# bigai-nlco/VideoTGB

Measured on AMD Instinct MI355X. Metric: clips/sec end-to-end VideoQA (96->8 frames), higher is better.
Workload: dtype bf16; 1 GPU; InstructBLIP-Vicuna-7B + TGB, T=96->8 of 32 frames, 224x224, greedy 16 new tokens (BASELINE.json configs[2]); inputs=resident in HBM when the timed region starts, global_batch=124, parallelism=clip-parallel x1 (no data-path collective), streams=1, weights=seeded N(0,0.02) random init

## Files before the change

### videotgb_amd/csrc/conv64.hip

```cpp
#include <type_traits>
#include <utility>
#include "common.h"
#include "pair_h8.h"

namespace {

constexpr int C64_R = 8, C64_RS = 128;
constexpr int C64_ROW_BYTES = C64_RS * 128;
constexpr int C64_LDS = C64_R * C64_ROW_BYTES + 8 * 32 * 2 * 4 + 64 * 4;
typedef __attribute__((address_space(3))) void* c64_lptr_t;

struct Conv64Params {
    const bf16_t* in;
    const bf16_t* w;
    const float* bias;
    float* out_f32;
    float* stats;
    float* stats_part;
    bf16_t* out_bf16;
    const bf16_t* resid;
    int n_img, H, W, relu, post_relu;
    int parts, rows_per_part;
};

template <int MODE>
__global__ __launch_bounds__(512) void conv3x3_c64_kernel(const Conv64Params p) {
#if defined(__HIP_DEVICE_COMPILE__)
    extern __shared__ __attribute__((aligned(16))) char ring[];
    float* const xch = reinterpret_cast<float*>(ring + C64_R * C64_ROW_BYTES);
    const int tid = threadIdx.x, lane = tid & 63, fr = lane & 15, fg = lane >> 4;
    const int wave = __builtin_amdgcn_readfirstlane(tid >> 6);
    const int wm = wave & 3, wn = wave >> 2;
    const int H = p.H, W = p.W;

    bf16x8 wf[9][2][2];
#pragma unroll
    for (int t = 0; t < 9; t++)
#pragma unroll
        for (int ks = 0; ks < 2; ks++)
#pragma unroll
            for (int i = 0; i < 2; i++)
                wf[t][ks][i] = *reinterpret_cast<const bf16x8*>(p.w + (wn * 32 + i * 16 + fr) * 576 + t * 64 + ks * 32 + fg * 8);
    float* const bias_s = xch + 8 * 32 * 2;
    if (tid < 64) bias_s[tid] = p.bias[tid];

    unsigned dma_off[2];
#pragma unroll
    for (int q = 0; q < 2; q++) {
        const int slot = (wave * 2 + q) * 8 + (lane >> 3), x = slot - 1, c = (lane & 7) ^ ((slot >> 1) & 7);
        dma_off[q] = (x >= 0 && x < W) ? (unsigned)(x * 64 + c * 8) * 2u : 0x80000000u;
    }
    unsigned x_off[3];
    int px[2];
#pragma unroll
    for (int j = 0; j < 2; j++) px[j] = wm * 32 + j * 16 + fr;
#pragma unroll
    for (int kx = 0; kx < 3; kx++) x_off[kx] = (unsigned)((px[0] + kx) * 128 + ((fg ^ (((px[0] + kx) >> 1) & 7)) << 4));

    typedef __attribute__((__vector_size__(4 * sizeof(unsigned)))) unsigned u32x4_t;
    typedef __attribute__((__vector_size__(2 * sizeof(unsigned)))) unsigned u32x2_t;
    constexpr unsigned OOB = 0x80000000u;
    constexpr int ES = MODE == 0 ? 4 : 2;
    unsigned o_off[2][2];
#pragma unroll
    for (int i = 0; i < 2; i++)
#pragma unroll
        for (int j = 0; j < 2; j++) o_off[i][j] = px[j] < W ? (unsigned)(px[j] * 64 + wn * 32 + i * 16 + fg * 4) * ES : OOB;

    const int n_units = p.n_img * p.parts;
    for (int unit = blockIdx.x; unit < n_units; unit += gridDim.x) {
        const int img = unit / p.parts, y0 = (unit - img * p.parts) * p.rows_per_part;
        if (y0 >= H) continue;
        const int y1 = y0 + p.rows_per_part < H ? y0 + p.rows_per_part : H;
        const bf16_t* const ibase = p.in + (int64_t)img * H * W * 64;
        const auto rsrc = __builtin_amdgcn_make_buffer_rsrc(const_cast<bf16_t*>(ibase), 0, H * W * 128, 0x00020000);
        const auto orsrc = __builtin_amdgcn_make_buffer_rsrc(MODE == 0 ? (void*)(p.out_f32 + (int64_t)img * H * W * 64) : (void*)(p.out_bf16 + (int64_t)img * H * W * 64), 0,
                                                             H * W * 64 * ES, 0x00020000);
        const auto rrsrc = __builtin_amdgcn_make_buffer_rsrc(const_cast<bf16_t*>(p.resid ? p.resid + (int64_t)img * H * W * 64 : ibase), 0, H * W * 128, 0x00020000);
#define C64_ISSUE(yy)                                                                                                          \
        {                                                                                                                      \
            const int so_ = ((yy) >= 0 && (yy) < H) ? (yy) * W * 128 : 0x7FFFFF00;        \
            char* const dst_ = ring + ((yy) & (C64_R - 1)) * C64_ROW_BYTES + (wave * 2) * 1024;                                \
            __builtin_amdgcn_raw_ptr_buffer_load_lds(rsrc, (c64_lptr_t)dst_, 16, dma_off[0], so_, 0, 0);                       \
            __builtin_amdgcn_raw_ptr_buffer_load_lds(rsrc, (c64_lptr_t)(dst_ + 1024), 16, dma_off[1], so_, 0, 0);              \
        }
        __builtin_amdgcn_s_waitcnt(0x0F70);
        __builtin_amdgcn_s_barrier();
        C64_ISSUE(y0 - 1)
        C64_ISSUE(y0)
        C64_ISSUE(y0 + 1)
        C64_ISSUE(y0 + 2)
        f32x4 s1[2] = {f32x4{0.f, 0.f, 0.f, 0.f}, f32x4{0.f, 0.f, 0.f, 0.f}}, s2[2] = {s1[0], s1[0]};
        for (int y = y0; y < y1; y += 2) {
            if (y == y0) __builtin_amdgcn_s_waitcnt(0x0F70);
            else __builtin_amdgcn_s_waitcnt(0x0F78);
            __builtin_amdgcn_s_barrier();
            bf16x4 rres[2][2][2];
            if constexpr (MODE == 1) {
                if (p.resid) {
#pragma unroll
                    for (int o = 0; o < 2; o++)
#pragma unroll
                        for (int i = 0; i < 2; i++)
#pragma unroll
                            for (int j = 0; j < 2; j++) {
                                const unsigned off = (y + o < y1 && o_off[i][j] != OOB) ? o_off[i][j] + (unsigned)((y + o) * W * 64 * 2) : OOB;
                                rres[o][i][j] = __builtin_bit_cast(bf16x4, __builtin_amdgcn_raw_buffer_load_b64(rrsrc, off, 0, 0));
                            }
                }
            }
            C64_ISSUE(y + 3)
            C64_ISSUE(y + 4)
            f32x4 acc[2][2][2];
#pragma unroll
            for (int o = 0; o < 2; o++)
#pragma unroll
                for (int i = 0; i < 2; i++)
#pragma unroll
                    for (int j = 0; j < 2; j++) acc[o][i][j] = f32x4{0.f, 0.f, 0.f, 0.f};
#pragma unroll
            for (int rr = 0; rr < 4; rr++) {
                const char* const rowp = ring + ((y + rr - 1) & (C64_R - 1)) * C64_ROW_BYTES;
#pragma unroll
                for (int kx = 0; kx < 3; kx++)
#pragma unroll
                    for (int ks = 0; ks < 2; ks++) {
                        const bf16x8 x0 = *reinterpret_cast<const bf16x8*>(rowp + (x_off[kx] ^ (ks * 64)));
                        const bf16x8 x1 = *reinterpret_cast<const bf16x8*>(rowp + (x_off[kx] ^ (ks * 64)) + 2048);
#pragma unroll
                        for (int o = 0; o < 2; o++) {
                            const int ky = rr - o;
                            if (ky < 0 || ky > 2) continue;
#pragma unroll
                            for (int i = 0; i < 2; i++) {
                                acc[o][i][0] = __builtin_amdgcn_mfma_f32_16x16x32_bf16(wf[ky * 3 + kx][ks][i], x0, acc[o][i][0], 0, 0, 0);
                                acc[o][i][1] = __builtin_amdgcn_mfma_f32_16x16x32_bf16(wf[ky * 3 + kx][ks][i], x1, acc[o][i][1], 0, 0, 0);
                            }
                        }
                    }
            }
            f32x4 b4[2];
#pragma unroll
            for (int i = 0; i < 2; i++) b4[i] = *reinterpret_cast<const f32x4*>(bias_s + wn * 32 + i * 16 + fg * 4);
#pragma unroll
            for (int o = 0; o < 2; o++) {
                const bool row_ok = y + o < y1;
#pragma unroll
                for (int i = 0; i < 2; i++)
#pragma unroll
                    for (int j = 0; j < 2; j++) {
                        const bool ok = row_ok && o_off[i][j] != OOB;
                        const unsigned off = ok ? o_off[i][j] + (unsigned)((y + o) * W * 64 * ES) : OOB;
                        f32x4 v = acc[o][i][j] + b4[i];
                        if constexpr (MODE == 0) {
                            __builtin_amdgcn_raw_buffer_store_b128(__builtin_bit_cast(u32x4_t, v), orsrc, off, 0, 0);
                            const f32x4 vz = {ok ? v[0] : 0.f, ok ? v[1] : 0.f, ok ? v[2] : 0.f, ok ? v[3] : 0.f};
                            s1[i] += vz;
                            s2[i] += vz * vz;
                        } else {
                            if (p.relu) v = f32x4{fmaxf(v[0], 0.f), fmaxf(v[1], 0.f), fmaxf(v[2], 0.f), fmaxf(v[3], 0.f)};
                            if (p.resid) {
                                const bf16x4 r = rres[o][i][j];
                                v += f32x4{(float)r[0], (float)r[1], (float)r[2], (float)r[3]};
                            }
                            if (p.post_relu) v = f32x4{fmaxf(v[0], 0.f), fmaxf(v[1], 0.f), fmaxf(v[2], 0.f), fmaxf(v[3], 0.f)};
                            const bf16x4 pk = {(bf16_t)v[0], (bf16_t)v[1], (bf16_t)v[2], (bf16_t)v[3]};
                            __builtin_amdgcn_raw_buffer_store_b64(__builtin_bit_cast(u32x2_t, pk), orsrc, off, 0, 0);
                        }
                    }
            }
        }
#undef C64_ISSUE
        if constexpr (MODE == 0) {
#pragma unroll
            for (int i = 0; i < 2; i++)
#pragma unroll
                for (int e = 0; e < 4; e++) {
                    float a_ = s1[i][e], b_ = s2[i][e];
#pragma unroll
                    for (int off = 1; off < 16; off <<= 1) { a_ += __shfl_xor(a_, off); b_ += __shfl_xor(b_, off); }
                    s1[i][e] = a_; s2[i][e] = b_;
                }
            __builtin_amdgcn_s_waitcnt(0xC07F);
            __builtin_amdgcn_s_barrier();
            if (fr == 0) {
#pragma unroll
                for (int i = 0; i < 2; i++)
#pragma unroll
                    for (int e = 0; e < 4; e++) {
                        xch[(wave * 32 + i * 16 + fg * 4 + e) * 2] = s1[i][e];
                        xch[(wave * 32 + i * 16 + fg * 4 + e) * 2 + 1] = s2[i][e];
                    }
            }
            __syncthreads();
            if (tid < 128) {
                const int ch = tid >> 1, which = tid & 1, wn_ = ch >> 5, c32 = ch & 31;
                float t = 0.f;
#pragma unroll
                for (int m_ = 0; m_ < 4; m_++) t += xch[((wn_ * 4 + m_) * 32 + c32) * 2 + which];
                if (p.parts == 1) p.stats[((int64_t)img * 64 + ch) * 2 + which] = t;
                else p.stats_part[((int64_t)unit * 64 + ch) * 2 + which] = t;
            }
        }
    }
#endif
}


constexpr int ST_R = 5;
struct StemParams {
    const float* img;
    const bf16_t* w;
    const float* bias;
    float* out_f32;
    float* stats;
    float* stats_part;
    bf16_t* out_bf16;
    int n_img, H, W, relu;
    int parts, rows_per_part;
    int h8;
};

template <int MODE, bool X3>
__global__ __launch_bounds__(512) void stem7x7_kernel(const StemParams p) {
    static_assert(X3 ? (MODE == 0 || MODE == 2) : (MODE == 0 || MODE == 1), "stem7x7: bf16 stores fp32 / bf16 rows, the split form fp32 / pair rows");
#if defined(__HIP_DEVICE_COMPILE__)
    extern __shared__ __attribute__((aligned(16))) char ring[];
    const int tid = threadIdx.x, lane = tid & 63, fr = lane & 15, fg = lane >> 4;
    const int wave = __builtin_amdgcn_readfirstlane(tid >> 6);
    const int wm = wave & 3, wn = wave >> 2;
    const int H = p.H, W = p.W, H2 = H >> 1, W2 = W >> 1;
    const int row_bytes = W2 * 256;
    float* const xch = reinterpret_cast<float*>(ring + ST_R * row_bytes);
    float* const bias_s = xch + 8 * 32 * 2;
    if (tid < 64) bias_s[tid] = p.bias[tid];
    for (int i = tid; i < ST_R * W2 * 4; i += 512) {
        const int pxl = i >> 2, X = pxl % W2, c = 6 + (i & 1) + ((i & 2) << 2);
        *reinterpret_cast<uint4*>(ring + pxl * 256 + ((c ^ (X & 15)) << 4)) = make_uint4(0, 0, 0, 0);
    }
    constexpr int W_LD = X3 ? 768 : 512;
    bf16x8 wf[16][2];
#pragma unroll
    for (int s_ = 0; s_ < 16; s_++)
#pragma unroll
        for (int i = 0; i < 2; i++)
            wf[s_][i] = *reinterpret_cast<const bf16x8*>(p.w + (wn * 32 + i * 16 + fr) * W_LD + (X3 ? (s_ >> 3) * 512 + (s_ & 7) * 32 : s_ * 32) + fg * 8);
    const bool builder = tid < W2 * 4;
    const int bX = tid >> 2, bdX = tid & 3, bcol = 2 * (bX + bdX - 2);
    const bool bcol_ok = builder && bcol >= 0 && bcol + 1 < W;
    const int bcol_c = bcol < 0 ? 0 : bcol + 1 < W ? bcol : W - 2;
    unsigned b_off[3];
#pragma unroll
    for (int q = 0; q < 3; q++) {
        const int off = bdX * 24 + q * 8;
        b_off[q] = (unsigned)(bX * 256 + (((off >> 4) ^ (bX & 15)) << 4) + (off & 8));
    }
    int px[2];
    unsigned x_off[2];
#pragma unroll
    for (int j = 0; j < 2; j++) {
        px[j] = wm * 32 + j * 16 + fr;
        const int pc = px[j] < W2 ? px[j] : 0;
        x_off[j] = (unsigned)(pc * 256 + ((fg ^ (pc & 15)) << 4));
    }
    typedef __attribute__((__vector_size__(4 * sizeof(unsigned)))) unsigned u32x4_t;
    typedef __attribute__((__vector_size__(2 * sizeof(unsigned)))) unsigned u32x2_t;
    constexpr unsigned OOB = 0x80000000u;
    constexpr int ES = MODE == 0 ? 4 : 2;
    constexpr int PXU = MODE == 2 ? 128 : 64;
    unsigned o_off[2][2];
#pragma unroll
    for (int i = 0; i < 2; i++)
#pragma unroll
        for (int j = 0; j < 2; j++) o_off[i][j] = px[j] < W2 ? (unsigned)(px[j] * PXU + wn * 32 + i * 16 + fg * 4) * ES : OOB;

    const int n_units = p.n_img * p.parts;
    for (int unit = blockIdx.x; unit < n_units; unit += gridDim.x) {
        const int img = unit / p.parts, y0 = (unit - img * p.parts) * p.rows_per_part;
        if (y0 >= H2) continue;
        const int y1 = y0 + p.rows_per_part < H2 ? y0 + p.rows_per_part : H2;
        const float* const ibase = p.img + (int64_t)img * 3 * H * W;
        const auto orsrc = __builtin_amdgcn_make_buffer_rsrc(MODE == 0 ? (void*)(p.out_f32 + (int64_t)img * H2 * W2 * 64) : (void*)(p.out_bf16 + (int64_t)img * H2 * W2 * PXU),
                                                             0, H2 * W2 * PXU * ES, 0x00020000);
        float2 ld[6];
#define ST_LOAD(Yp)       \
        {                                                                                                    \
            const int yc_ = (Yp) < 0 ? 0 : (Yp) >= H2 ? H2 - 1 : (Yp);                                       \
            _Pragma("unroll") for (int py = 0; py < 2; py++)                                                 \
                _Pragma("unroll") for (int c = 0; c < 3; c++)                                                \
                    ld[py * 3 + c] = *reinterpret_cast<const float2*>(ibase + ((int64_t)c * H + 2 * yc_ + py) * W + bcol_c); \
        }
#define ST_WRITE(Yp)                                                                                         \
        if (builder) {                                                                                       \
            const bool in_ = bcol_ok && (Yp) >= 0 && (Yp) < H2;                                              \
            bf16_t hi[12], lo[12];                                                                           \
            _Pragma("unroll") for (int py = 0; py < 2; py++)                                                 \
                _Pragma("unroll") for (int c = 0; c < 3; c++) {                                              \
                    const float d0 = in_ ? ld[py * 3 + c].x - 127.5f : 0.f, d1 = in_ ? ld[py * 3 + c].y - 127.5f : 0.f; \
                    const float h0_ = bf16_round(d0), h1_ = bf16_round(d1);                                  \
                    hi[py * 6 + c] = (bf16_t)h0_; lo[py * 6 + c] = (bf16_t)(d0 - h0_);                       \
                    hi[py * 6 + 3 + c] = (bf16_t)h1_; lo[py * 6 + 3 + c] = (bf16_t)(d1 - h1_);               \
                }                                                                                            \
            char* const rb_ = ring + ((((Yp) % ST_R) + ST_R) % ST_R) * row_bytes;                            \
            _Pragma("unroll") for (int q = 0; q < 3; q++) {                                                  \
                *reinterpret_cast<bf16x4*>(rb_ + b_off[q]) = bf16x4{hi[q * 4], hi[q * 4 + 1], hi[q * 4 + 2], hi[q * 4 + 3]}; \
                *reinterpret_cast<bf16x4*>(rb_ + (b_off[q] ^ 128)) = bf16x4{lo[q * 4], lo[q * 4 + 1], lo[q * 4 + 2], lo[q * 4 + 3]}; \
            }                                                                                                \
        }
        __syncthreads();
        for (int yy = y0 - 2; yy <= y0 + 1; yy++) {
            ST_LOAD(yy)
            ST_WRITE(yy)
        }
        f32x4 s1[2] = {f32x4{0.f, 0.f, 0.f, 0.f}, f32x4{0.f, 0.f, 0.f, 0.f}}, s2[2] = {s1[0], s1[0]};
        for (int y = y0; y < y1; y++) {
            __builtin_amdgcn_sched_barrier(0);
            __builtin_amdgcn_s_waitcnt(0xC07F);
            __builtin_amdgcn_s_barrier();
            __builtin_amdgcn_sched_barrier(0);
            ST_LOAD(y + 2)
            f32x4 acc[2][2], b4[2];
#define ST_STEP(tY, hl, half, s_)                                                                            \
            {                                                                                                \
                const char* const rowp = ring + ((y + (tY) - 2 + ST_R) % ST_R) * row_bytes;                  \
                const unsigned cx = (unsigned)(((hl) * 8 + (half) * 4) << 4);       \
                const bf16x8 x0 = *reinterpret_cast<const bf16x8*>(rowp + (x_off[0] ^ cx));                  \
                const bf16x8 x1 = *reinterpret_cast<const bf16x8*>(rowp + (x_off[1] ^ cx));                  \
                _Pragma("unroll") for (int i = 0; i < 2; i++) {                                              \
                    acc[i][0] = __builtin_amdgcn_mfma_f32_16x16x32_bf16(wf[s_][i], x0, acc[i][0], 0, 0, 0);  \
                    acc[i][1] = __builtin_amdgcn_mfma_f32_16x16x32_bf16(wf[s_][i], x1, acc[i][1], 0, 0, 0);  \
                }                                                                                            \
            }
            if constexpr (X3) {
#pragma unroll
                for (int i = 0; i < 2; i++) b4[i] = *reinterpret_cast<const f32x4*>(bias_s + wn * 32 + i * 16 + fg * 4);
#pragma unroll
                for (int i = 0; i < 2; i++)
#pragma unroll
                    for (int j = 0; j < 2; j++) acc[i][j] = b4[i] + f32x4{0.f, 0.f, 0.f, 0.f};
#pragma unroll
                for (int c = 0; c < 3; c++) {
#pragma unroll
                    for (int tY = 0; tY < 4; tY++)
#pragma unroll
                        for (int half = 0; half < 2; half++) ST_STEP(tY, c == 1 ? 1 : 0, half, (c == 2 ? 8 : 0) + tY * 2 + half)
                    if (c < 2) __builtin_amdgcn_sched_barrier(0);
                }
            } else {
#pragma unroll
                for (int i = 0; i < 2; i++)
#pragma unroll
                    for (int j = 0; j < 2; j++) acc[i][j] = f32x4{0.f, 0.f, 0.f, 0.f};
#pragma unroll
                for (int tY = 0; tY < 4; tY++)
#pragma unroll
                    for (int hl = 0; hl < 2; hl++)
#pragma unroll
                        for (int half = 0; half < 2; half++) ST_STEP(tY, hl, half, hl * 8 + tY * 2 + half)
#pragma unroll
                for (int i = 0; i < 2; i++) b4[i] = *reinterpret_cast<const f32x4*>(bias_s + wn * 32 + i * 16 + fg * 4);
            }
#undef ST_STEP
#pragma unroll
            for (int i = 0; i < 2; i++)
#pragma unroll
                for (int j = 0; j < 2; j++) {
                    const bool ok = o_off[i][j] != OOB;
                    const unsigned off = ok ? o_off[i][j] + (unsigned)(y * W2 * PXU * ES) : OOB;
                    f32x4 v = X3 ? acc[i][j] : acc[i][j] + b4[i];
                    if constexpr (MODE == 0) {
                        __builtin_amdgcn_raw_buffer_store_b128(__builtin_bit_cast(u32x4_t, v), orsrc, off, 0, 0);
                        const f32x4 vz = {ok ? v[0] : 0.f, ok ? v[1] : 0.f, ok ? v[2] : 0.f, ok ? v[3] : 0.f};
                        s1[i] += vz;
                        s2[i] += vz * vz;
                    } else if constexpr (MODE == 2) {
                        if (p.relu) v = f32x4{fmaxf(v[0], 0.f), fmaxf(v[1], 0.f), fmaxf(v[2], 0.f), fmaxf(v[3], 0.f)};
                        u32x2_t hu, lu;
                        if (p.h8) {
                            h8_split4(v, hu, lu);
                        } else {
                            bf16x4 hi, lo;
                            pair_split4(v, hi, lo);
                            hu = __builtin_bit_cast(u32x2_t, hi); lu = __builtin_bit_cast(u32x2_t, lo);
                        }
                        __builtin_amdgcn_raw_buffer_store_b64(hu, orsrc, off, 0, 0);
                        __builtin_amdgcn_raw_buffer_store_b64(lu, orsrc, ok ? off + 128u : OOB, 0, 0);
                    } else {
                        if (p.relu) v = f32x4{fmaxf(v[0], 0.f), fmaxf(v[1], 0.f), fmaxf(v[2], 0.f), fmaxf(v[3], 0.f)};
                        const bf16x4 pk = {(bf16_t)v[0], (bf16_t)v[1], (bf16_t)v[2], (bf16_t)v[3]};
                        __builtin_amdgcn_raw_buffer_store_b64(__builtin_bit_cast(u32x2_t, pk), orsrc, off, 0, 0);
                    }
                }
            ST_WRITE(y + 2)
        }
#undef ST_LOAD
#undef ST_WRITE
        if constexpr (X3) {
            if (!p.stats) continue;
        }
        if constexpr (MODE == 0) {
#pragma unroll
            for (int i = 0; i < 2; i++)
#pragma unroll
                for (int e = 0; e < 4; e++) {
                    float a_ = s1[i][e], b_ = s2[i][e];
#pragma unroll
                    for (int off = 1; off < 16; off <<= 1) { a_ += __shfl_xor(a_, off); b_ += __shfl_xor(b_, off); }
                    s1[i][e] = a_; s2[i][e] = b_;
                }
            __syncthreads();
            if (fr == 0) {
#pragma unroll
                for (int i = 0; i < 2; i++)
#pragma unroll
                    for (int e = 0; e < 4; e++) {
                        xch[(wave * 32 + i * 16 + fg * 4 + e) * 2] = s1[i][e];
                        xch[(wave * 32 + i * 16 + fg * 4 + e) * 2 + 1] = s2[i][e];
                    }
            }
            __syncthreads();
            if (tid < 128) {
                const int ch = tid >> 1, which = tid & 1, wn_ = ch >> 5, c32 = ch & 31;
                float t = 0.f;
#pragma unroll
                for (int m_ = 0; m_ < 4; m_++) t += xch[((wn_ * 4 + m_) * 32 + c32) * 2 + which];
                if (p.parts == 1) p.stats[((int64_t)img * 64 + ch) * 2 + which] = t;
                else p.stats_part[((int64_t)unit * 64 + ch) * 2 + which] = t;
            }
        }
    }
#endif
}

constexpr int L1_R = 4;
constexpr int L1_MAX_W = 112;
constexpr int L1_READ_SPAN = 130 * 256;
typedef int l1_i32x4 __attribute__((ext_vector_type(4)));
typedef int l1_i32x8 __attribute__((ext_vector_type(8)));
typedef _Float16 l1_f16x8 __attribute__((ext_vector_type(8)));

template <class F, int... G>
__device__ __forceinline__ void l1_static_for(std::integer_sequence<int, G...>, F&& f) { (f(std::integral_constant<int, G>{}), ...); }

struct Layer1H8Params {
    const char* in;
    const char* w;
    const float* bias;
    const int* scale;
    float* out_f32;
    char* out_pair;
    const char* resid;
    int n_img, H, W, out_bf16;
    int parts, rows_per_part, row_bytes;
};

template <int MODE, int OBF>
__global__ __launch_bounds__(512) void layer1_h8_kernel(const Layer1H8Params p) {
#if defined(__HIP_DEVICE_COMPILE__)
    extern __shared__ __attribute__((aligned(16))) char ring[];
    const int tid = threadIdx.x, lane = tid & 63, fr = lane & 15, fg = lane >> 4;
    const int wave = __builtin_amdgcn_readfirstlane(tid >> 6);
    const int wn = wave & 3, wm = wave >> 2;
    const int H = p.H, W = p.W, row_bytes = p.row_bytes;
    const int sc_w = *p.scale;

    l1_i32x4 wh[9][2];
    l1_i32x8 wc[9];
    {
        const char* const wrow = p.w + (wn * 16 + fr) * 2304 + fg * 16;
#pragma unroll
        for (int t = 0; t < 9; t++) {
            wh[t][0] = *reinterpret_cast<const l1_i32x4*>(wrow + t * 128);
            wh[t][1] = *reinterpret_cast<const l1_i32x4*>(wrow + t * 128 + 64);
            wc[t].lo = *reinterpret_cast<const l1_i32x4*>(wrow + (9 + t) * 128);
            wc[t].hi = *reinterpret_cast<const l1_i32x4*>(wrow + (9 + t) * 128 + 64);
        }
    }
    float* const bias_s = reinterpret_cast<float*>(ring + (L1_R - 1) * row_bytes + L1_READ_SPAN);
    if (tid < 64) bias_s[tid] = p.bias[tid];
    __syncthreads();

    constexpr unsigned OOB = 0x80000000u;
    const int n_pieces = row_bytes >> 10;
    const int dma_x = wave * 4 + (lane >> 4) - 1;
    const unsigned dma_off0 = (unsigned)(dma_x * 256 + (((lane & 15) ^ ((dma_x + 1) & 15)) << 4));
    unsigned x_off[3];
#pragma unroll
    for (int kx = 0; kx < 3; kx++) {
        const int slot = wm * 64 + fr + kx;
        x_off[kx] = (unsigned)(slot * 256 + ((fg ^ (slot & 15)) << 4));
    }
    const int nj = W - wm * 64 >= 64 ? 4 : W - wm * 64 <= 0 ? 0 : (W - wm * 64 + 15) >> 4;
    typedef __attribute__((__vector_size__(4 * sizeof(unsigned)))) unsigned u32x4_t;
    typedef __attribute__((__vector_size__(2 * sizeof(unsigned)))) unsigned u32x2_t;
    constexpr int OPX = 256;
    constexpr int OCH = MODE == 0 ? 4 : 2;
    const int px0 = wm * 64 + fr;
    const unsigned o_off0 = (unsigned)(px0 * OPX + (wn * 16 + fg * 4) * OCH);

    const int n_units = p.n_img * p.parts;
    for (int unit = blockIdx.x; unit < n_units; unit += gridDim.x) {
        const int img = unit / p.parts, y0 = (unit - img * p.parts) * p.rows_per_part;
        if (y0 >= H) continue;
        const int y1 = y0 + p.rows_per_part < H ? y0 + p.rows_per_part : H;
        const int64_t ioff = (int64_t)img * H * W * 256;
        const auto rsrc = __builtin_amdgcn_make_buffer_rsrc(const_cast<char*>(p.in + ioff), 0, H * W * 256, 0x00020000);
        const auto orsrc = __builtin_amdgcn_make_buffer_rsrc(MODE == 0 ? (void*)(reinterpret_cast<char*>(p.out_f32) + ioff) : (void*)(p.out_pair + ioff), 0, H * W * OPX, 0x00020000);
        const auto rrsrc = __builtin_amdgcn_make_buffer_rsrc(const_cast<char*>((MODE == 2 ? p.resid : p.in) + ioff), 0, H * W * 256, 0x00020000);
#define L1_ISSUE(yy)                                                                                                          \
        {                                                                                                                      \
            const int so_ = ((yy) >= 0 && (yy) < H) ? (yy) * W * 256 : 0x7FFFFF00;        \
            char* const dst_ = ring + ((yy) & (L1_R - 1)) * row_bytes + wave * 1024;                                           \
            _Pragma("unroll") for (int q = 0; q < 4; q++)                                                                      \
                if (q * 8 + wave < n_pieces)                                                                                   \
                    __builtin_amdgcn_raw_ptr_buffer_load_lds(rsrc, (c64_lptr_t)(dst_ + q * 8192), 16,                          \
                                                             (dma_x + q * 32 >= 0 && dma_x + q * 32 < W) ? dma_off0 + q * 8192u : OOB, so_, 0, 0); \
        }
        __builtin_amdgcn_s_waitcnt(0x0F70);
        __builtin_amdgcn_s_barrier();
        L1_ISSUE(y0 - 1)
        L1_ISSUE(y0)
        L1_ISSUE(y0 + 1)
        auto step = [&](auto nj_c, const int y) {
            constexpr int NJ = decltype(nj_c)::value;
            constexpr int NST = (MODE == 0 ? 1 : 2) * NJ;
            if (y == y0) __builtin_amdgcn_s_waitcnt(0x0F70);
            else __builtin_amdgcn_s_waitcnt(0x0F70 | NST);
            __builtin_amdgcn_s_barrier();
            u32x2_t rh[NJ], rl[NJ];
            if constexpr (MODE == 2) {
#pragma unroll
                for (int jj = 0; jj < NJ; jj++) {
                    const unsigned off = px0 + jj * 16 < W ? o_off0 + (unsigned)(jj * 16 * OPX + y * W * 256) : OOB;
                    rh[jj] = __builtin_bit_cast(u32x2_t, __builtin_amdgcn_raw_buffer_load_b64(rrsrc, off, 0, 0));
                    rl[jj] = __builtin_bit_cast(u32x2_t, __builtin_amdgcn_raw_buffer_load_b64(rrsrc, off != OOB ? off + 128u : OOB, 0, 0));
                }
            }
            L1_ISSUE(y + 2)
            f32x4 acc[NJ];
#pragma unroll
            for (int jj = 0; jj < NJ; jj++) acc[jj] = *reinterpret_cast<const f32x4*>(bias_s + wn * 16 + fg * 4);
            l1_i32x4 xg[3][NJ];
#define L1_READ(g)                                                                                                             \
            {                                                                                                                  \
                constexpr int t_ = (g) < 18 ? (g) / 2 : ((g) - 18) / 2;                                                        \
                constexpr unsigned cx_ = (g) < 18 ? ((g) & 1) * 64u : 128u + ((g) & 1) * 64u;                                  \
                const char* const rowp_ = ring + ((y + t_ / 3 - 1) & (L1_R - 1)) * row_bytes;                                  \
                _Pragma("unroll") for (int jj = 0; jj < NJ; jj++)                                                              \
                    xg[(g) % 3][jj] = *reinterpret_cast<const l1_i32x4*>(rowp_ + (x_off[t_ % 3] ^ cx_) + jj * 4096);           \
            }
            L1_READ(0)
            __builtin_amdgcn_sched_barrier(0);
            l1_static_for(std::make_integer_sequence<int, 36>{}, [&](auto gc) {
                constexpr int g = decltype(gc)::value;
                if constexpr (g + 1 < 36) { L1_READ(g + 1) }
                if constexpr (g < 18) {
#pragma unroll
                    for (int jj = 0; jj < NJ; jj++)
                        acc[jj] = __builtin_amdgcn_mfma_f32_16x16x32_f16(__builtin_bit_cast(l1_f16x8, wh[g / 2][g & 1]), __builtin_bit_cast(l1_f16x8, xg[g % 3][jj]), acc[jj], 0, 0, 0);
                } else if constexpr ((g & 1) != 0) {
#pragma unroll
                    for (int jj = 0; jj < NJ; jj++) {
                        l1_i32x8 xc;
                        xc.lo = xg[(g - 1) % 3][jj]; xc.hi = xg[g % 3][jj];
                        acc[jj] = __builtin_amdgcn_mfma_scale_f32_16x16x128_f8f6f4(wc[(g - 18) / 2], xc, acc[jj], 0, 1, 0, sc_w, 0, 127);
                    }
                }
                if constexpr (g + 1 < 36) __builtin_amdgcn_sched_group_barrier(0x100, NJ, 0);
                if constexpr (g < 18 || (g & 1) != 0) __builtin_amdgcn_sched_group_barrier(0x008, NJ, 0);
                __builtin_amdgcn_sched_barrier(0);
            });
#undef L1_READ
            __builtin_amdgcn_sched_barrier(0);
#pragma unroll
            for (int jj = 0; jj < NJ; jj++) {
                const bool ok = px0 + jj * 16 < W;
                const unsigned off = ok ? o_off0 + (unsigned)(jj * 16 * OPX + y * W * OPX) : OOB;
                f32x4 v = acc[jj];
                if constexpr (MODE == 0) {
                    __builtin_amdgcn_raw_buffer_store_b128(__builtin_bit_cast(u32x4_t, v), orsrc, off, 0, 0);
                } else {
                    v = f32x4{fmaxf(v[0], 0.f), fmaxf(v[1], 0.f), fmaxf(v[2], 0.f), fmaxf(v[3], 0.f)};
                    if constexpr (MODE == 2) {
                        v += h8_join4(rh[jj], rl[jj]);
                        v = f32x4{fmaxf(v[0], 0.f), fmaxf(v[1], 0.f), fmaxf(v[2], 0.f), fmaxf(v[3], 0.f)};
                    }
                    u32x2_t hu, lu;
                    if constexpr (OBF) {
                        bf16x4 hi, lo;
                        pair_split4(v, hi, lo);
                        hu = __builtin_bit_cast(u32x2_t, hi); lu = __builtin_bit_cast(u32x2_t, lo);
                    } else {
                        h8_split4(v, hu, lu);
                    }
                    __builtin_amdgcn_raw_buffer_store_b64(hu, orsrc, off, 0, 0);
                    __builtin_amdgcn_raw_buffer_store_b64(lu, orsrc, ok ? off + 128u : OOB, 0, 0);
                }
            }
        };
        if (nj == 3) {
            for (int y = y0; y < y1; y++) step(std::integral_constant<int, 3>{}, y);
        } else {
            for (int y = y0; y < y1; y++) step(std::integral_constant<int, 4>{}, y);
        }
#undef L1_ISSUE
    }
#endif
}

}

bool conv3x3_c64_supported(int H, int W) { return W >= 16 && W <= C64_RS - 2 && H >= 1; }

size_t conv64_stats_part_floats(int n_img) { return ((size_t)n_img + 4 * (size_t)cu_count()) * 2 * 64 * 2; }

int launch_conv3x3_c64(const void* in, const void* w, const float* bias, float* out_f32, float* stats, float* stats_part, void* out_bf16, const void* resid,
                       int n_img, int H, int W, int relu, int post_relu, hipStream_t s) {
    VTGB_REQUIRE(conv3x3_c64_supported(H, W), VTGB_EUNSUPPORTED, "conv3x3_c64: W=%d outside [16, %d]", W, C64_RS - 2);
    VTGB_REQUIRE((int64_t)H * W * 128 < 0x7FFFFF00ll, VTGB_EUNSUPPORTED, "conv3x3_c64: image too large");
    Conv64Params p;
    p.in = (const bf16_t*)in; p.w = (const bf16_t*)w; p.bias = bias; p.out_f32 = out_f32; p.stats = stats; p.stats_part = stats_part; p.out_bf16 = (bf16_t*)out_bf16;
    p.resid = (const bf16_t*)resid; p.n_img = n_img; p.H = H; p.W = W; p.relu = relu; p.post_relu = post_relu;
    int parts = 1;
    while ((int64_t)n_img * parts < 4 * cu_count() && H / (parts * 2) >= 8) parts *= 2;
    p.rows_per_part = 2 * ((H + 2 * parts - 1) / (2 * parts));
    p.parts = (H + p.rows_per_part - 1) / p.rows_per_part;
    const int64_t units = (int64_t)n_img * p.parts;
    const int grid = units < cu_count() ? (int)units : cu_count();
    if (out_f32 && p.parts > 1) VTGB_REQUIRE(stats_part && (size_t)units * 128 <= conv64_stats_part_floats(n_img), VTGB_EINVAL, "conv3x3_c64: partial-moment scratch missing");
    const double flops = 2.0 * n_img * H * W * 64.0 * 576.0;
    ProfScope prof(VTGB_PROF_CONV, flops, s, flops);
    static DeviceOnce a0, a1;
    if (out_f32) {
        VTGB_REQUIRE(stats, VTGB_EINVAL, "conv3x3_c64: fp32 output needs the moments buffer");
        VTGB_FUNC_LDS_ONCE(a0, conv3x3_c64_kernel<0>, C64_LDS);
        hipLaunchKernelGGL(conv3x3_c64_kernel<0>, dim3(grid), dim3(512), C64_LDS, s, p);
        if (p.parts > 1) VTGB_TRY(launch_stats_finish_parts(stats_part, stats, n_img, p.parts, 64, s));
    } else {
        VTGB_FUNC_LDS_ONCE(a1, conv3x3_c64_kernel<1>, C64_LDS);
        hipLaunchKernelGGL(conv3x3_c64_kernel<1>, dim3(grid), dim3(512), C64_LDS, s, p);
    }
    VTGB_HIP(hipGetLastError());
    return VTGB_OK;
}

bool stem7x7_supported(int H, int W) { return (H % 2) == 0 && (W % 2) == 0 && W / 2 >= 16 && W / 2 <= 112 && H / 2 >= 4; }

static int stem7x7_launch(bool x3, const float* img, const void* w, const float* bias, float* out_f32, float* stats, float* stats_part, void* out16, int h8, int n_img,
                          int H, int W, int relu, hipStream_t s) {
    VTGB_REQUIRE(stem7x7_supported(H, W), VTGB_EUNSUPPORTED, "stem7x7: %d x %d unsupported", H, W);
    const int H2 = H / 2, W2 = W / 2;
    VTGB_REQUIRE((int64_t)H2 * W2 * 256 < 0x7FFFFF00ll, VTGB_EUNSUPPORTED, "stem7x7: image too large");
    StemParams p;
    p.img = img; p.w = (const bf16_t*)w; p.bias = bias; p.out_f32 = out_f32; p.stats = stats; p.stats_part = stats_part; p.out_bf16 = (bf16_t*)out16;
    p.n_img = n_img; p.H = H; p.W = W; p.relu = relu; p.h8 = h8;
    int parts = 1;
    while ((int64_t)n_img * parts < 4 * cu_count() && H2 / (parts * 2) >= 14) parts *= 2;
    p.rows_per_part = (H2 + parts - 1) / parts;
    p.parts = (H2 + p.rows_per_part - 1) / p.rows_per_part;
    const int64_t units = (int64_t)n_img * p.parts;
    const int grid = units < cu_count() ? (int)units : cu_count();
    if (out_f32 && stats && p.parts > 1)
        VTGB_REQUIRE(stats_part && (size_t)units * 128 <= conv64_stats_part_floats(n_img), VTGB_EINVAL, "stem7x7: partial-moment scratch missing");
    const int lds = ST_R * W2 * 256 + 8 * 32 * 2 * 4 + 64 * 4;
    constexpr int lds_max = ST_R * 112 * 256 + 8 * 32 * 2 * 4 + 64 * 4;
    const double flops = 2.0 * n_img * H2 * W2 * 64.0 * 147.0, exec = 2.0 * n_img * H2 * W2 * 64.0 * (x3 ? 768.0 : 512.0);
    ProfScope prof(VTGB_PROF_CONV, flops, s, exec);
    static DeviceOnce a0, a1, a2, a3;
    if (out_f32) {
        VTGB_REQUIRE(stats || x3, VTGB_EINVAL, "stem7x7: fp32 output needs the moments buffer");
        if (x3) {
            VTGB_FUNC_LDS_ONCE(a2, (stem7x7_kernel<0, true>), lds_max);
            hipLaunchKernelGGL((stem7x7_kernel<0, true>), dim3(grid), dim3(512), lds, s, p);
        } else {
            VTGB_FUNC_LDS_ONCE(a0, (stem7x7_kernel<0, false>), lds_max);
            hipLaunchKernelGGL((stem7x7_kernel<0, false>), dim3(grid), dim3(512), lds, s, p);
        }
        if (stats && p.parts > 1) VTGB_TRY(launch_stats_finish_parts(stats_part, stats, n_img, p.parts, 64, s));
    } else if (x3) {
        VTGB_FUNC_LDS_ONCE(a3, (stem7x7_kernel<2, true>), lds_max);
        hipLaunchKernelGGL((stem7x7_kernel<2, true>), dim3(grid), dim3(512), lds, s, p);
    } else {
        VTGB_FUNC_LDS_ONCE(a1, (stem7x7_kernel<1, false>), lds_max);
        hipLaunchKernelGGL((stem7x7_kernel<1, false>), dim3(grid), dim3(512), lds, s, p);
    }
    VTGB_HIP(hipGetLastError());
    return VTGB_OK;
}

int launch_stem7x7(const float* img, const void* w, const float* bias, float* out_f32, float* stats, float* stats_part, void* out_bf16, int n_img, int H, int W,
                   int relu, hipStream_t s) {
    return stem7x7_launch(false, img, w, bias, out_f32, stats, stats_part, out_bf16, 0, n_img, H, W, relu, s);
}
int launch_stem7x7_x3(const float* img, const void* w, const float* bias, float* out_f32, float* stats, float* stats_part, void* out_pair, int h8, int n_img, int H,
                      int W, hipStream_t s) {
    VTGB_REQUIRE((out_f32 != nullptr) != (out_pair != nullptr), VTGB_EINVAL, "stem7x7 x3: exactly one of the fp32 rows and the pair rows");
    return stem7x7_launch(true, img, w, bias, out_f32, stats, stats_part, out_pair, h8, n_img, H, W, out_pair ? 1 : 0, s);
}

bool layer1_h8_supported(int H, int W) { return W >= 16 && W <= L1_MAX_W && H >= 4 && (int64_t)H * W * 256 < 0x7FFFFF00ll; }

int launch_layer1_h8(const void* in, const void* w, const float* bias, const int* scale, float* out_f32, void* out_pair, const void* resid, int out_bf16, int n_img, int H,
                     int W, hipStream_t s) {
    VTGB_REQUIRE(n_img > 0 && layer1_h8_supported(H, W), VTGB_EUNSUPPORTED, "layer1_h8: %d images of %d x %d outside 16 <= W <= %d, H >= 4", n_img, H, W, L1_MAX_W);
    VTGB_REQUIRE(in && w && bias && scale && ((out_f32 != nullptr) != (out_pair != nullptr)) && (!resid || out_pair) && (!out_bf16 || resid), VTGB_EINVAL,
                 "layer1_h8: operands, the scale byte and exactly one of the fp32 rows and the pair rows (resid belongs to pair rows, bf16 pairs to the residual tail)");
    Layer1H8Params p;
    p.in = (const char*)in; p.w = (const char*)w; p.bias = bias; p.scale = scale; p.out_f32 = out_f32; p.out_pair = (char*)out_pair; p.resid = (const char*)resid;
    p.n_img = n_img; p.H = H; p.W = W; p.out_bf16 = out_bf16;
    p.row_bytes = ((W + 2 + 3) / 4) * 1024;
    int parts = 1;
    while ((int64_t)n_img * parts < 4 * cu_count() && H / (parts * 2) >= 7) parts *= 2;
    p.rows_per_part = (H + parts - 1) / parts;
    p.parts = (H + p.rows_per_part - 1) / p.rows_per_part;
    const int64_t units = (int64_t)n_img * p.parts;
    const int grid = units < cu_count() ? (int)units : cu_count();
    const int lds = (L1_R - 1) * p.row_bytes + L1_READ_SPAN + 256;
    constexpr int lds_max = (L1_R - 1) * ((L1_MAX_W + 2 + 3) / 4) * 1024 + L1_READ_SPAN + 256;
    const double flops = 2.0 * n_img * H * W * 64.0 * 576.0;
    ProfScope prof(VTGB_PROF_CONV, flops, s, 2.0 * flops);
    static DeviceOnce a0, a1, a2, a3;
    if (out_f32) {
        VTGB_FUNC_LDS_ONCE(a0, (layer1_h8_kernel<0, 0>), lds_max);
        hipLaunchKernelGGL((layer1_h8_kernel<0, 0>), dim3(grid), dim3(512), lds, s, p);
    } else if (!resid) {
        VTGB_FUNC_LDS_ONCE(a1, (layer1_h8_kernel<1, 0>), lds_max);
        hipLaunchKernelGGL((layer1_h8_kernel<1, 0>), dim3(grid), dim3(512), lds, s, p);
    } else if (!out_bf16) {
        VTGB_FUNC_LDS_ONCE(a2, (layer1_h8_kernel<2, 0>), lds_max);
        hipLaunchKernelGGL((layer1_h8_kernel<2, 0>), dim3(grid), dim3(512), lds, s, p);
    } else {
        VTGB_FUNC_LDS_ONCE(a3, (layer1_h8_kernel<2, 1>), lds_max);
        hipLaunchKernelGGL((layer1_h8_kernel<2, 1>), dim3(grid), dim3(512), lds, s, p);
    }
    VTGB_HIP(hipGetLastError());
    return VTGB_OK;
}
```

Before: 38.67 clips/s.

## Add 4-wave layer1 h8 conv kernel for the non-residual modes

```diff
diff --git a/videotgb_amd/csrc/conv64.hip b/videotgb_amd/csrc/conv64.hip
--- a/videotgb_amd/csrc/conv64.hip
+++ b/videotgb_amd/csrc/conv64.hip
@@ -597,6 +597,149 @@
                     __builtin_amdgcn_raw_buffer_store_b64(lu, orsrc, ok ? off + 128u : OOB, 0, 0);
                 }
             }
+        };
+        if (nj == 3) {
+            for (int y = y0; y < y1; y++) step(std::integral_constant<int, 3>{}, y);
+        } else {
+            for (int y = y0; y < y1; y++) step(std::integral_constant<int, 4>{}, y);
+        }
+#undef L1_ISSUE
+    }
+#endif
+}
+
+constexpr int l1_waitcnt_vm(int n) { return 0x0F70 | (n & 15) | ((n >> 4) << 14); }
+
+template <int MODE>
+__global__ __launch_bounds__(256) __attribute__((amdgpu_waves_per_eu(1, 1))) void layer1_h8_w4_kernel(const Layer1H8Params p) {
+    static_assert(MODE == 0 || MODE == 1, "layer1_h8_w4: fp32 rows or relu(.) as an f16c8 pair (the residual tail runs on layer1_h8_kernel)");
+#if defined(__HIP_DEVICE_COMPILE__)
+    extern __shared__ __attribute__((aligned(16))) char ring[];
+    const int tid = threadIdx.x, lane = tid & 63, fr = lane & 15, fg = lane >> 4;
+    const int wave = __builtin_amdgcn_readfirstlane(tid >> 6);
+    const int cp = wave & 1, wm = wave >> 1;
+    const int H = p.H, W = p.W, row_bytes = p.row_bytes;
+    const int sc_w = *p.scale;
+
+    l1_i32x4 wh[2][9][2];
+    l1_i32x8 wc[2][9];
+    f32x4 bias[2];
+#pragma unroll
+    for (int b = 0; b < 2; b++) {
+        const char* const wrow = p.w + (cp * 32 + b * 16 + fr) * 2304 + fg * 16;
+#pragma unroll
+        for (int t = 0; t < 9; t++) {
+            wh[b][t][0] = *reinterpret_cast<const l1_i32x4*>(wrow + t * 128);
+            wh[b][t][1] = *reinterpret_cast<const l1_i32x4*>(wrow + t * 128 + 64);
+            wc[b][t].lo = *reinterpret_cast<const l1_i32x4*>(wrow + (9 + t) * 128);
+            wc[b][t].hi = *reinterpret_cast<const l1_i32x4*>(wrow + (9 + t) * 128 + 64);
+        }
+        bias[b] = *reinterpret_cast<const f32x4*>(p.bias + cp * 32 + b * 16 + fg * 4);
+    }
+
+    constexpr unsigned OOB = 0x80000000u;
+    const int n_pieces = row_bytes >> 10;
+    const int dma_x = wave * 4 + (lane >> 4) - 1;
+    const unsigned dma_off0 = (unsigned)(dma_x * 256 + (((lane & 15) ^ ((dma_x + 1) & 15)) << 4));
+    unsigned x_off[3];
+#pragma unroll
+    for (int kx = 0; kx < 3; kx++) {
+        const int slot = wm * 64 + fr + kx;
+        x_off[kx] = (unsigned)(slot * 256 + ((fg ^ (slot & 15)) << 4));
+    }
+    const int nj = W - wm * 64 >= 64 ? 4 : W - wm * 64 <= 0 ? 0 : (W - wm * 64 + 15) >> 4;
+    typedef __attribute__((__vector_size__(4 * sizeof(unsigned)))) unsigned u32x4_t;
+    typedef __attribute__((__vector_size__(2 * sizeof(unsigned)))) unsigned u32x2_t;
+    constexpr int OPX = 256;
+    constexpr int OCH = MODE == 0 ? 4 : 2;
+    const int px0 = wm * 64 + fr;
+    const unsigned o_off0 = (unsigned)(px0 * OPX + (cp * 32 + fg * 4) * OCH);
+
+    const int n_units = p.n_img * p.parts;
+    for (int unit = blockIdx.x; unit < n_units; unit += gridDim.x) {
+        const int img = unit / p.parts, y0 = (unit - img * p.parts) * p.rows_per_part;
+        if (y0 >= H) continue;
+        const int y1 = y0 + p.rows_per_part < H ? y0 + p.rows_per_part : H;
+        const int64_t ioff = (int64_t)img * H * W * 256;
+        const auto rsrc = __builtin_amdgcn_make_buffer_rsrc(const_cast<char*>(p.in + ioff), 0, H * W * 256, 0x00020000);
+        const auto orsrc = __builtin_amdgcn_make_buffer_rsrc(MODE == 0 ? (void*)(reinterpret_cast<char*>(p.out_f32) + ioff) : (void*)(p.out_pair + ioff), 0, H * W * OPX, 0x00020000);
+#define L1_ISSUE(yy)                                                                                                          \
+        {                                                                                                                      \
+            const int so_ = ((yy) >= 0 && (yy) < H) ? (yy) * W * 256 : 0x7FFFFF00;        \
+            char* const dst_ = ring + ((yy) & (L1_R - 1)) * row_bytes + wave * 1024;                                           \
+            _Pragma("unroll") for (int q = 0; q < 8; q++)                                                                     \
+                if (q * 4 + wave < n_pieces)                                                                                   \
+                    __builtin_amdgcn_raw_ptr_buffer_load_lds(rsrc, (c64_lptr_t)(dst_ + q * 4096), 16,                          \
+                                                             (dma_x + q * 16 >= 0 && dma_x + q * 16 < W) ? dma_off0 + q * 4096u : OOB, so_, 0, 0); \
+        }
+        __builtin_amdgcn_s_waitcnt(0x0F70);
+        __builtin_amdgcn_s_barrier();
+        L1_ISSUE(y0 - 1)
+        L1_ISSUE(y0)
+        L1_ISSUE(y0 + 1)
+        auto step = [&](auto nj_c, const int y) {
+            constexpr int NJ = decltype(nj_c)::value;
+            constexpr int NST = (MODE == 0 ? 1 : 2) * 2 * NJ;
+            if (y == y0) __builtin_amdgcn_s_waitcnt(0x0F70);
+            else __builtin_amdgcn_s_waitcnt(l1_waitcnt_vm(NST));
+            __builtin_amdgcn_s_barrier();
+            L1_ISSUE(y + 2)
+            f32x4 acc[2][NJ];
+#pragma unroll
+            for (int jj = 0; jj < NJ; jj++) { acc[0][jj] = bias[0]; acc[1][jj] = bias[1]; }
+            l1_i32x4 xg[3][NJ];
+#define L1_READ(g)                                                                                                             \
+            {                                                                                                                  \
+                constexpr int t_ = (g) < 18 ? (g) / 2 : ((g) - 18) / 2;                                                        \
+                constexpr unsigned cx_ = (g) < 18 ? ((g) & 1) * 64u : 128u + ((g) & 1) * 64u;                                  \
+                const char* const rowp_ = ring + ((y + t_ / 3 - 1) & (L1_R - 1)) * row_bytes;                                  \
+                _Pragma("unroll") for (int jj = 0; jj < NJ; jj++)                                                              \
+                    xg[(g) % 3][jj] = *reinterpret_cast<const l1_i32x4*>(rowp_ + (x_off[t_ % 3] ^ cx_) + jj * 4096);           \
+            }
+            L1_READ(0)
+            __builtin_amdgcn_sched_barrier(0);
+            l1_static_for(std::make_integer_sequence<int, 36>{}, [&](auto gc) {
+                constexpr int g = decltype(gc)::value;
+                if constexpr (g + 1 < 36) { L1_READ(g + 1) }
+                if constexpr (g < 18) {
+#pragma unroll
+                    for (int jj = 0; jj < NJ; jj++)
+#pragma unroll
+                        for (int b = 0; b < 2; b++)
+                            acc[b][jj] = __builtin_amdgcn_mfma_f32_16x16x32_f16(__builtin_bit_cast(l1_f16x8, wh[b][g / 2][g & 1]), __builtin_bit_cast(l1_f16x8, xg[g % 3][jj]), acc[b][jj], 0, 0, 0);
+                } else if constexpr ((g & 1) != 0) {
+#pragma unroll
+                    for (int jj = 0; jj < NJ; jj++) {
+                        l1_i32x8 xc;
+                        xc.lo = xg[(g - 1) % 3][jj]; xc.hi = xg[g % 3][jj];
+#pragma unroll
+                        for (int b = 0; b < 2; b++)
+                            acc[b][jj] = __builtin_amdgcn_mfma_scale_f32_16x16x128_f8f6f4(wc[b][(g - 18) / 2], xc, acc[b][jj], 0, 1, 0, sc_w, 0, 127);
+                    }
+                }
+                if constexpr (g + 1 < 36) __builtin_amdgcn_sched_group_barrier(0x100, NJ, 0);
+                if constexpr (g < 18 || (g & 1) != 0) __builtin_amdgcn_sched_group_barrier(0x008, 2 * NJ, 0);
+                __builtin_amdgcn_sched_barrier(0);
+            });
+#undef L1_READ
+            __builtin_amdgcn_sched_barrier(0);
+#pragma unroll
+            for (int jj = 0; jj < NJ; jj++)
+#pragma unroll
+                for (int b = 0; b < 2; b++) {
+                    const bool ok = px0 + jj * 16 < W;
+                    const unsigned off = ok ? o_off0 + (unsigned)(b * 16 * OCH + jj * 16 * OPX + y * W * OPX) : OOB;
+                    f32x4 v = acc[b][jj];
+                    if constexpr (MODE == 0) {
+                        __builtin_amdgcn_raw_buffer_store_b128(__builtin_bit_cast(u32x4_t, v), orsrc, off, 0, 0);
+                    } else {
+                        v = f32x4{fmaxf(v[0], 0.f), fmaxf(v[1], 0.f), fmaxf(v[2], 0.f), fmaxf(v[3], 0.f)};
+                        u32x2_t hu, lu;
+                        h8_split4(v, hu, lu);
+                        __builtin_amdgcn_raw_buffer_store_b64(hu, orsrc, off, 0, 0);
+                        __builtin_amdgcn_raw_buffer_store_b64(lu, orsrc, ok ? off + 128u : OOB, 0, 0);
+                    }
+                }
         };
         if (nj == 3) {
             for (int y = y0; y < y1; y++) step(std::integral_constant<int, 3>{}, y);
@@ -721,11 +864,11 @@
     ProfScope prof(VTGB_PROF_CONV, flops, s, 2.0 * flops);
     static DeviceOnce a0, a1, a2, a3;
     if (out_f32) {
-        VTGB_FUNC_LDS_ONCE(a0, (layer1_h8_kernel<0, 0>), lds_max);
-        hipLaunchKernelGGL((layer1_h8_kernel<0, 0>), dim3(grid), dim3(512), lds, s, p);
+        VTGB_FUNC_LDS_ONCE(a0, layer1_h8_w4_kernel<0>, lds_max);
+        hipLaunchKernelGGL(layer1_h8_w4_kernel<0>, dim3(grid), dim3(256), lds, s, p);
     } else if (!resid) {
-        VTGB_FUNC_LDS_ONCE(a1, (layer1_h8_kernel<1, 0>), lds_max);
-        hipLaunchKernelGGL((layer1_h8_kernel<1, 0>), dim3(grid), dim3(512), lds, s, p);
+        VTGB_FUNC_LDS_ONCE(a1, layer1_h8_w4_kernel<1>, lds_max);
+        hipLaunchKernelGGL(layer1_h8_w4_kernel<1>, dim3(grid), dim3(256), lds, s, p);
     } else if (!out_bf16) {
         VTGB_FUNC_LDS_ONCE(a2, (layer1_h8_kernel<2, 0>), lds_max);
         hipLaunchKernelGGL((layer1_h8_kernel<2, 0>), dim3(grid), dim3(512), lds, s, p);
```

New measurement: 38.77 clips/s (median of 6 runs). Within noise of the previous version (+0.3%).
